# geonuklee/slam-toolkit

Measured on NVIDIA B200. Metric: orb_extract_match_stereo_frames_per_s, higher is better.
Workload: dtype u8

## Files before the change

slam-toolkit_b200/csrc/sfe_extract.cu:

```cuda
#include <cuda_fp16.h>

#include <algorithm>
#include <cmath>
#include <mutex>
#include <type_traits>

#include "sfe_extract.cuh"

namespace sfe {

__device__ __forceinline__ uint32_t ldg_word_at(const uint8_t *p) {
    const uintptr_t a = (uintptr_t)p;
    const uint32_t *w = (const uint32_t *)(a & ~(uintptr_t)3);
    return __funnelshift_r(__ldg(w), __ldg(w + 1), (uint32_t)(a & 3) * 8);
}

__device__ __forceinline__ uint32_t dp4a_u8u8(uint32_t a, uint32_t b, uint32_t c) {
    uint32_t d;
    asm("dp4a.u32.u32 %0, %1, %2, %3;" : "=r"(d) : "r"(a), "r"(b), "r"(c));
    return d;
}
__device__ __forceinline__ uint32_t dp2a_lo(uint32_t a, uint32_t b, uint32_t c) {
    uint32_t d;
    asm("dp2a.lo.u32.u32 %0, %1, %2, %3;" : "=r"(d) : "r"(a), "r"(b), "r"(c));
// ... 130 lines not shown
    uint32_t p[16], lo3[16], hi3[16];
#pragma unroll
    for (int k = 0; k < 16; k++) p[k] = __byte_perm(c0[off[k]], c1[off[k]], 0x5410);
#pragma unroll
    for (int s = 0; s < 16; s++) {
        lo3[s] = __vimin3_s16x2(p[s], p[(s + 1) & 15], p[(s + 2) & 15]);
        hi3[s] = __vimax3_s16x2(p[s], p[(s + 1) & 15], p[(s + 2) & 15]);
    }
    uint32_t max_of_min = 0u, min_of_max = 0x7fff7fffu;
#pragma unroll
    for (int s = 0; s < 16; s += 2) {
        const uint32_t l0 = __vimin3_s16x2(lo3[s], lo3[(s + 3) & 15], lo3[(s + 6) & 15]);
        const uint32_t l1 = __vimin3_s16x2(lo3[s + 1], lo3[(s + 4) & 15], lo3[(s + 7) & 15]);
        const uint32_t h0 = __vimax3_s16x2(hi3[s], hi3[(s + 3) & 15], hi3[(s + 6) & 15]);
        const uint32_t h1 = __vimax3_s16x2(hi3[s + 1], hi3[(s + 4) & 15], hi3[(s + 7) & 15]);
        max_of_min = __vimax3_s16x2(max_of_min, l0, l1);
        min_of_max = __vimin3_s16x2(min_of_max, h0, h1);
    }
    const int v0 = c0[0], v1 = c1[0];
    best0 = max(v0 - (int)(min_of_max & 0xFFFF), (int)(max_of_min & 0xFFFF) - v0);
    best1 = max(v1 - (int)(min_of_max >> 16), (int)(max_of_min >> 16) - v1);
}

template <bool kTma>
__global__ void __launch_bounds__(kFastThreads, kFastCtasPerSm) fast_segments_kernel(ImgSet S, FastPlan P, const SegRec *__restrict__ segs,
                                                                     const __grid_constant__ TmaMaps M) {
    constexpr int TP = kFastTilePitch, TW = TP / 4, SP = kFastScorePitch, T = kFastThreads;
    pdl_enter();
    extern __shared__ __align__(128) uint32_t fast_smem[];
    uint32_t *tile32 = fast_smem;
    uint8_t *score = (uint8_t *)(tile32 + P.tile_rows * TW);
    uint16_t *pre = (uint16_t *)(score + P.score_rows * SP);
    uint16_t *det = pre + P.list_cap;
    __shared__ int n_pre, n_det;
    __shared__ int cell_surv[kFastMaxCells];
    __shared__ uint64_t bar;
    const uint8_t *tile = (const uint8_t *)tile32;

    const uint4 rec = __ldg((const uint4 *)segs + blockIdx.x);
    const int ini_x = (short)(rec.x & 0xFFFF), ini_y = (short)(rec.x >> 16), tw = (short)(rec.y & 0xFFFF);
    const int sh = (rec.y >> 16) & 0xFF, level = rec.y >> 24, n_cells = rec.z & 0xFF, w_cell = (rec.z >> 8) & 0xFF;
    const int inv_w = rec.z >> 16, th = sh - 6;
    const FastLevel &F = P.lv[level];
    const int img = blockIdx.y, tid = threadIdx.x, lane = tid & 31, warp = tid >> 5;
    const int xa = (ini_x - 4) & ~15;
    const int cs = ini_x + 3 - xa;
    if (kTma) {
        if (tid == 0) {
            mbar_init(&bar, 1);
            mbar_expect_tx(&bar, (uint32_t)(P.tile_rows * TP));
            const bool set_a = img < S.split;
            const CUtensorMap *map = level == 0 ? (set_a ? &M.lv[0] : &M.l0b) : &M.lv[level];
            const int z = level == 0 ? S.in_z0 + (set_a ? img : img - S.split) : slot_of(S, img);
            tma_load_3d(tile32, map, &bar, xa, ini_y, z);
        }
    } else {
        const uint8_t *src;
        int pitch;
        if (level == 0) {
            pitch = S.in_pitch;
            src = img < S.split ? S.in_a + (size_t)img * S.in_stride : S.in_b + (size_t)(img - S.split) * S.in_stride;
        } else {
            pitch = F.pitch;
            src = S.pyr + (size_t)slot_of(S, img) * S.pyr_stride + F.plane_off;
        }
        src += (size_t)ini_y * pitch + xa;
        const int nw = min(((cs + tw - 1) >> 2) + 2, TW);
        for (int r = warp; r < sh; r += T / 32)
            for (int j = lane; j < nw; j += 32) tile32[r * TW + j] = ldg_word_at(src + (size_t)r * pitch + 4 * j);
    }
    const int jw = (cs >> 2) + lane, x0 = 4 * jw - cs;
    uint32_t vm = 0;
#pragma unroll
    for (int k = 0; k < 4; k++)
        if (x0 + k >= 0 && x0 + k < tw) vm |= 0x80u << (8 * k);
    uint32_t todo = (1u << n_cells) - 1;
    int t = P.ini_th;
    for (int i = tid; i < (th + 2) * (SP / 16); i += T) ((uint4 *)score)[i] = make_uint4(0, 0, 0, 0);
    for (int attempt = 0; attempt < 2; attempt++) {
        if (tid == 0) { n_pre = 0; n_det = 0; }
        if (tid < kFastMaxCells) cell_surv[tid] = 0;
        __syncthreads();
        if (kTma && attempt == 0) mbar_wait(&bar, 0);
        uint32_t vm_now = vm;
        if (attempt) {
#pragma unroll
            for (int k = 0; k < 4; k++)
                if (!((todo >> ((max(x0 + k, 0) * inv_w) >> 16)) & 1)) vm_now &= ~(0x80u << (8 * k));
        }
        const uint32_t kk = (uint32_t)(0x7F - min(t, 127)) * 0x01010101u;
        if (vm_now) {
            const uint32_t *row = tile32 + (warp + 3) * TW + jw;
            for (int y = warp; y < th; y += T / 32, row += (T / 32) * TW) {
                const uint32_t c = row[0];
                const uint32_t dv0 = __vabsdiffu4(row[-3 * TW], c), dv1 = __vabsdiffu4(row[3 * TW], c);
                const uint32_t dh0 = __vabsdiffu4(__byte_perm(row[-1], c, 0x4321), c);
                const uint32_t dh1 = __vabsdiffu4(__byte_perm(c, row[1], 0x6543), c);
                const uint32_t rv = (((dv0 | dv1) & 0x7F7F7F7Fu) + kk) | dv0 | dv1;
                const uint32_t rh = (((dh0 | dh1) & 0x7F7F7F7Fu) + kk) | dh0 | dh1;
                const uint32_t m = rv & rh & vm_now;
                if (m) {
                    int pos = atomicAdd(&n_pre, __popc(m));
                    const uint16_t item = (uint16_t)((y << 8) + x0);
                    if (m & 0x80u) pre[pos++] = item;
                    if (m & 0x8000u) pre[pos++] = item + 1;
                    if (m & 0x800000u) pre[pos++] = item + 2;
                    if (m & 0x80000000u) pre[pos] = item + 3;
                }
            }
        }
        __syncthreads();
        const int np = n_pre, npairs = (np + 1) >> 1;
        for (int e0 = 0; e0 < npairs; e0 += T) {
            bool corner0 = false, corner1 = false;
            uint16_t yx0 = 0, yx1 = 0;
            const int e = e0 + tid;
            if (e < npairs) {
                yx0 = pre[2 * e];
                yx1 = pre[min(2 * e + 1, np - 1)];
                int best0, best1;
                fast_best_x2<TP>(&tile[((yx0 >> 8) + 3) * TP + (yx0 & 255) + cs], &tile[((yx1 >> 8) + 3) * TP + (yx1 & 255) + cs],
                                 best0, best1);
                corner0 = best0 > t;
                corner1 = best1 > t && 2 * e + 1 < np;
                if (corner0) score[((yx0 >> 8) + 1) * SP + (yx0 & 255) + 1] = (uint8_t)best0;
                if (corner1) score[((yx1 >> 8) + 1) * SP + (yx1 & 255) + 1] = (uint8_t)best1;
            }
            const uint32_t c0 = __ballot_sync(0xffffffffu, corner0), c1 = __ballot_sync(0xffffffffu, corner1);
            if (c0 | c1) {
                int base = 0;
                if (lane == 0) base = atomicAdd(&n_det, __popc(c0) + __popc(c1));
                base = __shfl_sync(0xffffffffu, base, 0);
                const uint32_t lt = (1u << lane) - 1;
                if (corner0) det[base + __popc(c0 & lt)] = yx0;
                if (corner1) det[base + __popc(c0) + __popc(c1 & lt)] = yx1;
            }
        }
        __syncthreads();
        const int nd = n_det, slot = slot_of(S, img);
        uint32_t *out = S.cand + (size_t)slot * S.cand_stride + F.cand_off;
        for (int e0 = warp * 32; e0 < nd; e0 += T) {
            bool keep = false;
            uint32_t packed = 0;
            int cell = 0;
            if (e0 + lane < nd) {
                const uint16_t yx = det[e0 + lane];
                const int x = yx & 255, y = yx >> 8;
                cell = (x * inv_w) >> 16;
                const int cx0 = cell * w_cell, cx1 = min(cx0 + w_cell, tw);
                const uint8_t *sc = &score[(y + 1) * SP + x + 1];
                const int s = sc[0];
                const int lft = x > cx0 ? __vimax3_s32(sc[-1], sc[-SP - 1], sc[SP - 1]) : 0;
                const int rgt = x + 1 < cx1 ? __vimax3_s32(sc[1], sc[-SP + 1], sc[SP + 1]) : 0;
                keep = s > __vimax3_s32(max(sc[-SP], sc[SP]), lft, rgt);
                packed = (uint32_t)(s - 1) << 24 | (uint32_t)(ini_y - kBorder + y + 3) << 12 | (uint32_t)(ini_x - kBorder + x + 3);
            }
            const uint32_t kept = __ballot_sync(0xffffffffu, keep);
            if (kept) {
                int base = 0;
                if (lane == 0) base = atomicAdd(&S.cand_count[slot * S.nlevels + level], __popc(kept));
                base = __shfl_sync(0xffffffffu, base, 0);
                if (keep) {
                    const int o = base + __popc(kept & ((1u << lane) - 1));
                    if (o < F.cand_cap) out[o] = packed;
                    else atomicOr(&S.flags[slot], kFlagCandOverflow);
                    cell_surv[cell] = 1;
                }
            }
        }
        __syncthreads();
        const uint32_t retry = __ballot_sync(0xffffffffu, lane < n_cells && ((todo >> lane) & 1) && cell_surv[min(lane, kFastMaxCells - 1)] == 0);
        if (retry == 0 || P.min_th >= t) break;
        t = P.min_th;
        todo = retry;
        __syncthreads();
    }
}

template <bool kWide>
struct ONodeT {
    typedef typename std::conditional<kWide, uint32_t, unsigned short>::type pos_t;
    short x0, x1, y0, y1;
    pos_t start, cnt;
};

template <bool kWide>
struct OctSmemT {
    typedef ONodeT<kWide> ONode;
    typedef typename ONode::pos_t pos_t;
    uint32_t *pk[2];
    uint16_t *own[2];
    pos_t *qs;
    ONode *nd[2];
    uint16_t *eidx[2];
    uint32_t *child;
    uint16_t *childpos;
    int *tord;
    int *arr_a, *arr_b;
// ... 886 lines not shown
    }
}

}

using namespace sfe;

enum { kStagePyramid, kStageFast, kStageQuadtree, kStageBlur, kStageDescribe, kStageStereo, kStageTrack, kNumStages };
constexpr int kOctreeSmemCand = 3072;
constexpr int kComputeStreams = 4;
constexpr int kMaxChunks = 16;

struct sfe_extractor {
    int device = 0;
    cudaStream_t stream = nullptr;
    cudaStream_t s_h2d = nullptr, s_d2h = nullptr;
    cudaStream_t extra[kComputeStreams - 1] = {};
    int n_compute = 3;
    cudaStream_t aux[3] = {nullptr, nullptr, nullptr};
    cudaEvent_t ev_fork[3] = {}, ev_join[3] = {};
    int dev_split = 3;
    bool split_small = false;
    int octree_ctas = 0;
    int sm_count = 148;
    bool piped_now = false;
    bool orient_tma = true;
    bool overlap_tail = true;
    bool tail_pending = false;
    int overlap_blur = 2;
    cudaEvent_t ev_start = nullptr;
    bool async_dev = false;
    cudaEvent_t ev_in[kMaxChunks] = {}, ev_done[kMaxChunks] = {};
    int chunks_override = 0;
    bool trace = false;
    cudaEvent_t tr_ev[3 * kMaxChunks + 1] = {};
    sfe_extractor_params prm{};
    float scale[kMaxLevels], inv_scale[kMaxLevels], sigma2[kMaxLevels], inv_sigma2[kMaxLevels];
    int quota[kMaxLevels];
    int max_images = 0;
    int w = 0, h = 0;
    LevelPlan lv[kMaxLevels];
    FastPlan fast{};
    alignas(64) TmaMaps fast_maps{}, blur_maps{}, pyr_maps{};
    alignas(64) OrientMaps orient_maps{};
    int pyr_box_w = 0, pyr_box_h = 0;
    bool tma_plan_ok = false, tma_disabled = false, tma_now = false;
    const void *l0_key[2] = {nullptr, nullptr};
    size_t l0_geom[4] = {0, 0, 0, 0};
    int pitch0 = 0;
    std::vector<SegRec> segs;
    int seg_level_start[kMaxLevels + 1] = {};
    DevBuf<SegRec> d_segs;
    size_t fast_smem = 0, pyr_smem = 0;
    int pyr_wide_h[kMaxLevels] = {};
    std::vector<TilePlan> tiles;
    size_t pyr_stride = 0, blur_stride = 0;
    int cand_stride = 0, kpst_stride = 0, max_cand = 0, max_nodes = 0;
    size_t octree_smem = 0;
    int octree_smem_cand = 0, octree_slots = 0, octree_cand_override = 0;
    struct GraphEntry {
        uint64_t plan_gen = 0;
        int frames = 0, cap = 0, stereo = 0, seen = 0;
        double sp[3] = {0, 0, 0};
        const void *ptr[7] = {};
        cudaGraphExec_t exec = nullptr;
        int64_t launches = 0;
        uint64_t used = 0;
    };
    std::vector<GraphEntry> graphs;
    uint64_t plan_gen = 0, graph_clock = 0;
    bool use_graphs = true;
    bool use_pdl = true;
    bool octree_ff = true;
    bool pdl_now = false;
    bool octree_wide = false;
// ... 199 lines not shown
            for (int ty = 0; ty < L.h; ty += kPyrTileH) {
                const int last = std::min(ty + kPyrTileH, L.h) - 1;
                const int span = (int)(ytab[L.ytab_off + last].x >> 16) - (int)(ytab[L.ytab_off + ty].x & 0xFFFF) + 1;
                max_src_rows = std::max(max_src_rows, span);
            }
        }
    }
    ex->pyr_stride = std::max<size_t>(pyr_off, 128);
    ex->blur_stride = std::max<size_t>(blur_off, 128);
    ex->cand_stride = std::max(cand_off, 1);
    ex->kpst_stride = std::max(kp_off, 1);
    ex->max_cand = (std::max(max_cand, 1) + 7) & ~7;
    ex->max_nodes = max_nodes;
    ex->pyr_smem = (size_t)max_src_rows * kPyrTileW * sizeof(uint16_t);
    ex->pyr_box_w = (int)align_up((size_t)max_src_cols, 16);
    ex->pyr_box_h = max_src_rows;
    SFE_REQUIRE(ex->pyr_smem + (size_t)ex->pyr_box_w * ex->pyr_box_h <= 48 * 1024 && ex->pyr_box_w <= 256 && ex->pyr_box_h <= 256,
                SFE_ERR_UNSUPPORTED, "scale factor too large for the pyramid tile");
    ex->fast.nlevels = nl;
    ex->fast.ini_th = ex->prm.ini_th_fast;
    ex->fast.min_th = ex->prm.min_th_fast;
    ex->fast.n_segs = (int)ex->segs.size();
    ex->fast.tile_rows = (max_sh + 1) & ~1;
    ex->fast.score_rows = max_sh - 4;
    ex->fast.list_cap = (max_list + 7) & ~7;
    ex->fast_smem = (size_t)ex->fast.tile_rows * kFastTilePitch + (size_t)ex->fast.score_rows * kFastScorePitch + 2 * 2 * (size_t)ex->fast.list_cap;
    SFE_REQUIRE(ex->fast_smem <= 200 * 1024, SFE_ERR_UNSUPPORTED, "FAST segment working set exceeds shared memory");
    ex->octree_smem_cand = std::min(ex->max_cand, ex->octree_cand_override > 0 ? ex->octree_cand_override : kOctreeSmemCand) & ~7;
    if (ex->octree_smem_cand < 8) ex->octree_smem_cand = 8;
    ex->octree_wide = ex->max_cand > kNarrowCandCap;
    const size_t oct_cand_bytes = ex->octree_wide ? 16 : 14, oct_node_bytes = ex->octree_wide ? sizeof(ONodeT<true>) : sizeof(ONodeT<false>);
    ex->octree_smem = (size_t)ex->octree_smem_cand * oct_cand_bytes + (size_t)max_nodes * (16 + 3 * 4 + 2 * oct_node_bytes + 2 * 2 + 8) + 32 * 4 + 64;
    SFE_REQUIRE(ex->octree_smem <= 227 * 1024, SFE_ERR_UNSUPPORTED, "quadtree working set exceeds shared memory");
    {
        int big_levels = 0;
        for (int l = 0; l < nl; l++) big_levels += ex->lv[l].cand_cap > ex->octree_smem_cand;
        ex->octree_slots = big_levels * ex->max_images;
    }
    SFE_CUDA(ex->d_octree_scratch.ensure(std::max<size_t>((size_t)ex->octree_slots * ex->max_cand * oct_cand_bytes, 16)));
    const int n = ex->max_images;
    SFE_CUDA(ex->d_pyr.ensure(ex->pyr_stride * n));
    SFE_CUDA(ex->d_blur.ensure(ex->blur_stride * n));
    SFE_CUDA(ex->d_cand.ensure((size_t)ex->cand_stride * n));
    SFE_CUDA(ex->d_kpst.ensure((size_t)ex->kpst_stride * n));
    SFE_CUDA(ex->d_counts.ensure((size_t)n * (2 * nl + 1) + 1));
    SFE_CUDA(cudaMemsetAsync(ex->d_counts.p, 0, sizeof(int) * ex->d_counts.n, ex->stream));
    SFE_CUDA(ex->d_tiles.ensure(std::max<size_t>(ex->tiles.size(), 1)));
    SFE_CUDA(ex->d_segs.ensure(std::max<size_t>(ex->segs.size(), 1)));
    if (!ex->segs.empty())
        SFE_CUDA(cudaMemcpyAsync(ex->d_segs.p, ex->segs.data(), sizeof(SegRec) * ex->segs.size(), cudaMemcpyHostToDevice, ex->stream));
    SFE_CUDA(ex->d_xtab.ensure(std::max<size_t>(xtab.size(), 1)));
    SFE_CUDA(ex->d_ytab.ensure(std::max<size_t>(ytab.size(), 1)));
    if (!ex->tiles.empty())
        SFE_CUDA(cudaMemcpyAsync(ex->d_tiles.p, ex->tiles.data(), sizeof(TilePlan) * ex->tiles.size(), cudaMemcpyHostToDevice, ex->stream));
    if (!xtab.empty()) {
        SFE_CUDA(cudaMemcpyAsync(ex->d_xtab.p, xtab.data(), sizeof(uint2) * xtab.size(), cudaMemcpyHostToDevice, ex->stream));
        SFE_CUDA(cudaMemcpyAsync(ex->d_ytab.p, ytab.data(), sizeof(uint2) * ytab.size(), cudaMemcpyHostToDevice, ex->stream));
    }
    SFE_CUDA(cudaStreamSynchronize(ex->stream));
    ex->tma_plan_ok = !ex->tma_disabled;
    for (int l = 0; l < nl && ex->tma_plan_ok; l++) {
        const LevelPlan &L = ex->lv[l];
        if (L.w < 8 || L.h < 8) ex->tma_plan_ok = false;
        if (l == 0 || !ex->tma_plan_ok) continue;
        ex->tma_plan_ok = tma_encode_u8_3d(&ex->fast_maps.lv[l], ex->d_pyr.p + L.plane_off, L.w, L.h, n, L.pitch, ex->pyr_stride,
                                           kFastTilePitch, ex->fast.tile_rows) &&
                          tma_encode_u8_3d(&ex->blur_maps.lv[l], ex->d_pyr.p + L.plane_off, L.w, L.h, n, L.pitch, ex->pyr_stride,
                                           kBlurInWords * 4, kBlurTileH + 6) &&
                          (nl < 2 || tma_encode_u8_3d(&ex->pyr_maps.lv[l], ex->d_pyr.p + L.plane_off, L.w, L.h, n, L.pitch, ex->pyr_stride,
                                                      ex->pyr_box_w, ex->pyr_box_h)) &&
                          tma_encode_u8_3d(&ex->orient_maps.ic[l], ex->d_pyr.p + L.plane_off, L.w, L.h, n, L.pitch, ex->pyr_stride,
// ... 97 lines not shown
        const bool ok = tma_encode_u8_3d(&ex->fast_maps.lv[0], a, L.w, L.h, n_a, pitch, stride, kFastTilePitch, ex->fast.tile_rows) &&
                        tma_encode_u8_3d(&ex->fast_maps.l0b, b, L.w, L.h, n_b, pitch, stride, kFastTilePitch, ex->fast.tile_rows) &&
                        tma_encode_u8_3d(&ex->blur_maps.lv[0], a, L.w, L.h, n_a, pitch, stride, kBlurInWords * 4, kBlurTileH + 6) &&
                        tma_encode_u8_3d(&ex->blur_maps.l0b, b, L.w, L.h, n_b, pitch, stride, kBlurInWords * 4, kBlurTileH + 6) &&
                        (ex->prm.nlevels < 2 ||
                         (tma_encode_u8_3d(&ex->pyr_maps.lv[0], a, L.w, L.h, n_a, pitch, stride, ex->pyr_box_w, ex->pyr_box_h) &&
                          tma_encode_u8_3d(&ex->pyr_maps.l0b, b, L.w, L.h, n_b, pitch, stride, ex->pyr_box_w, ex->pyr_box_h))) &&
                        tma_encode_u8_3d(&ex->orient_maps.ic[0], a, L.w, L.h, n_a, pitch, stride, kIcBoxW, kIcBoxH) &&
                        tma_encode_u8_3d(&ex->orient_maps.ic_l0b, b, L.w, L.h, n_b, pitch, stride, kIcBoxW, kIcBoxH);
        ex->l0_key[0] = ok ? a : nullptr;
        ex->l0_key[1] = ok ? b : nullptr;
        memcpy(ex->l0_geom, geom, sizeof(geom));
        if (!ok) return;
    }
    ex->tma_now = true;
}

constexpr bool kFastTma = true;

static int launch_fast(sfe_extractor *ex, cudaStream_t st, const ImgSet &S, int count, int level0 = 0, int level1 = kMaxLevels) {
    level1 = std::min(level1, ex->prm.nlevels);
    const int seg0 = ex->seg_level_start[level0], nseg = ex->seg_level_start[level1] - seg0;
    if (nseg <= 0) return SFE_OK;
    const dim3 grid((unsigned)nseg, count);
    if (ex->fast_smem > 48 * 1024) {
        static std::mutex mu;
        static size_t granted[64] = {};
        std::lock_guard<std::mutex> lock(mu);
        if (ex->fast_smem > granted[ex->device & 63]) {
            SFE_CUDA(cudaFuncSetAttribute(fast_segments_kernel<true>, cudaFuncAttributeMaxDynamicSharedMemorySize, (int)ex->fast_smem));
            SFE_CUDA(cudaFuncSetAttribute(fast_segments_kernel<false>, cudaFuncAttributeMaxDynamicSharedMemorySize, (int)ex->fast_smem));
            granted[ex->device & 63] = ex->fast_smem;
        }
    }
    {
        static std::once_flag once[64];
        std::call_once(once[ex->device & 63], [] {
            cudaFuncSetAttribute(fast_segments_kernel<true>, cudaFuncAttributePreferredSharedMemoryCarveout, cudaSharedmemCarveoutMaxShared);
            cudaFuncSetAttribute(fast_segments_kernel<false>, cudaFuncAttributePreferredSharedMemoryCarveout, cudaSharedmemCarveoutMaxShared);
        });
    }
    if (ex->tma_now && kFastTma)
        launch_k(fast_segments_kernel<true>, grid, kFastThreads, ex->fast_smem, st, ex->pdl_now, S, ex->fast, ex->d_segs.p + seg0, ex->fast_maps);
    else
        launch_k(fast_segments_kernel<false>, grid, kFastThreads, ex->fast_smem, st, ex->pdl_now, S, ex->fast, ex->d_segs.p + seg0, ex->fast_maps);
    return SFE_OK;
}

constexpr int kSplitMaxImages = 4;

static int join_tail(sfe_extractor *ex) {
    if (ex->tail_pending) {
        SFE_CUDA(cudaStreamWaitEvent(ex->stream, ex->ev_join[1], 0));
        ex->tail_pending = false;
    }
    return SFE_OK;
}

static int enqueue_extract(sfe_extractor *ex, cudaStream_t st, const ImgSet &S, int count, const OutSet &O) {
    const int nl = ex->prm.nlevels;
    prof_mark(ex, 0);
    auto launch_pyr = [&](int l) {
        const LevelPlan &D = ex->lv[l], &Q = ex->lv[l - 1];
        const PyrStep P{D.w, D.h, D.pitch, D.plane_off, Q.w, l == 1 ? S.in_pitch : Q.pitch, Q.plane_off, l == 1, D.xtab_off, D.ytab_off,
                        l - 1, ex->pyr_box_w, ex->pyr_box_h, ex->pyr_wide_h[l]};
        dim3 grid(div_up(D.w, kPyrTileW), div_up(D.h, kPyrTileH), count);
        if (ex->tma_now)
            launch_k(pyr_resize_kernel<true>, grid, 256, ex->pyr_smem + (size_t)ex->pyr_box_w * ex->pyr_box_h, st, ex->pdl_now, S, P, ex->d_xtab.p,
// ... 536 lines not shown
        set_error("stream/event creation: %s", cudaGetErrorString(cudaGetLastError()));
        sfe_extractor_destroy(ex);
        return SFE_ERR_CUDA;
    }
    if (const char *env = getenv("SFE_PIPELINE_CHUNKS")) ex->chunks_override = atoi(env);
    if (const char *env = getenv("SFE_NO_TMA")) ex->tma_disabled = atoi(env) != 0;
    if (const char *env = getenv("SFE_OVERLAP_BLUR")) ex->overlap_blur = atoi(env);
    cudaDeviceGetAttribute(&ex->sm_count, cudaDevAttrMultiProcessorCount, device);
    if (const char *env = getenv("SFE_OCTREE_CTAS")) ex->octree_ctas = atoi(env);
    if (const char *env = getenv("SFE_ORIENT_TMA")) ex->orient_tma = atoi(env) != 0;
    if (const char *env = getenv("SFE_OVERLAP_TAIL")) ex->overlap_tail = atoi(env) != 0;
    if (const char *env = getenv("SFE_TRACE")) ex->trace = atoi(env) != 0;
    if (const char *env = getenv("SFE_COMPUTE_STREAMS")) ex->n_compute = std::max(1, std::min(atoi(env), kComputeStreams));
    if (ex->trace)
        for (auto &e : ex->tr_ev) cudaEventCreate(&e);
    if (const char *env = getenv("SFE_OCTREE_SMEM_CAND")) ex->octree_cand_override = atoi(env);
    if (const char *env = getenv("SFE_CAND_CAP")) ex->cand_cap_override = std::max(8, atoi(env));
    if (const char *env = getenv("SFE_GRAPHS")) ex->use_graphs = atoi(env) != 0;
    if (const char *env = getenv("SFE_PDL")) ex->use_pdl = atoi(env) != 0;
    if (const char *env = getenv("SFE_OCTREE_FF")) ex->octree_ff = atoi(env) != 0;
    if (const char *env = getenv("SFE_COPY_KERNEL")) ex->use_copy_kernel = atoi(env) != 0;
    if (const char *env = getenv("SFE_SPLIT_SMALL")) ex->split_small = atoi(env) != 0;
    if (const char *env = getenv("SFE_DEV_SPLIT")) ex->dev_split = std::max(1, std::min(atoi(env), kComputeStreams));
    build_tables(ex);
    *out = ex;
    return SFE_OK;
}

int sfe_extractor_destroy(sfe_extractor *ex) {
    if (!ex) return SFE_OK;
    drop_graphs(ex);
    if (ex->h_flags_pinned) cudaFreeHost(ex->h_flags_pinned);
    if (ex->h_stage) cudaFreeHost(ex->h_stage);
    DeviceGuard g(ex->device);
    SFE_REQUIRE(g.ok, SFE_ERR_NO_DEVICE, "cannot select the handle's device");
    cudaStreamSynchronize(ex->stream);
    ex->d_pyr.release(); ex->d_blur.release(); ex->d_in.release(); ex->d_l0.release(); ex->d_octree_scratch.release(); ex->d_desc.release();
    ex->d_cand.release(); ex->d_kpst.release(); ex->d_counts.release();
    ex->d_tiles.release(); ex->d_segs.release(); ex->d_xtab.release(); ex->d_ytab.release();
    ex->d_kps.release(); ex->d_nout.release(); ex->d_sidx.release(); ex->d_sdist.release(); ex->d_tidx.release(); ex->d_tdist.release();
    ex->track.cell_start.release(); ex->track.order.release(); ex->track.valid.release(); ex->track.sxy.release(); ex->track.sdesc.release(); ex->track.best.release();
    for (int i = 0; i <= kNumStages; i++)
        if (ex->prof_ev[i]) cudaEventDestroy(ex->prof_ev[i]);
    for (int i = 0; i < kMaxChunks; i++) {
        if (ex->ev_in[i]) cudaEventDestroy(ex->ev_in[i]);
        if (ex->ev_done[i]) cudaEventDestroy(ex->ev_done[i]);
    }
    for (auto &e : ex->tr_ev)
        if (e) cudaEventDestroy(e);
    for (int i = 0; i < 3; i++) {
        if (ex->ev_fork[i]) cudaEventDestroy(ex->ev_fork[i]);
        if (ex->ev_join[i]) cudaEventDestroy(ex->ev_join[i]);
        if (ex->aux[i]) cudaStreamDestroy(ex->aux[i]);
    }
    if (ex->ev_start) cudaEventDestroy(ex->ev_start);
    for (auto &e : ex->extra)
        if (e) cudaStreamDestroy(e);
    if (ex->s_h2d) cudaStreamDestroy(ex->s_h2d);
    if (ex->s_d2h) cudaStreamDestroy(ex->s_d2h);
    cudaStreamDestroy(ex->stream);
    delete ex;
    return SFE_OK;
// ... 105 lines not shown
    int rc = sfe_extract_batch(ex, image, (size_t)stride * (h > 0 ? h : 0), 1, w, h, stride, kps, desc, cap, &n);
    *n_out = n;
    return rc;
}

static int stereo_frames_dev_once(sfe_extractor *ex, const uint8_t *left_dev, const uint8_t *right_dev, size_t image_stride,
                                  int frames, int w, int h, int stride, const sfe_stereo_params *sp, const sfe_track_params *tp,
                                  sfe_keypoint *kps_l_dev, uint8_t *desc_l_dev, int32_t *n_l_dev, sfe_keypoint *kps_r_dev,
                                  uint8_t *desc_r_dev, int32_t *n_r_dev, int32_t *stereo_idx_dev, int32_t *stereo_dist_dev,
                                  int32_t *track_idx_dev, int32_t *track_dist_dev, int cap) {
    int rc = prepare(ex, 2 * frames, w, h, stride, cap);
    if (rc != SFE_OK) return rc;
    if (!sp) sp = &k_default_stereo;
    const OutSet O{kps_l_dev, kps_r_dev, desc_l_dev, desc_r_dev, n_l_dev, n_r_dev, cap};
    const ImgSet S = make_imgset(ex, left_dev, right_dev, frames, image_stride, stride);
    prepare_l0_maps(ex, left_dev, right_dev, frames, frames, image_stride, stride);
    if ((rc = reset_counters(ex)) != SFE_OK) return rc;
    const int nsplit = !ex->profiling && frames >= 16 * ex->dev_split ? std::min(ex->dev_split, ex->n_compute) : 1;
    if (nsplit <= 1) {
        if ((rc = enqueue_extract(ex, ex->stream, S, 2 * frames, O)) != SFE_OK) return rc;
    } else {
        SFE_CUDA(cudaEventRecord(ex->ev_start, ex->stream));
        for (int c = 1; c < nsplit; c++) SFE_CUDA(cudaStreamWaitEvent(ex->extra[c - 1], ex->ev_start, 0));
        for (int c = nsplit - 1; c >= 0; c--) {
            const int f0 = (int)((long long)frames * c / nsplit), f1 = (int)((long long)frames * (c + 1) / nsplit);
            cudaStream_t sc = c == 0 ? ex->stream : ex->extra[c - 1];
            if ((rc = enqueue_extract(ex, sc, chunk_of(S, f0, f1, true), 2 * (f1 - f0), chunk_of(O, f0))) != SFE_OK) return rc;
            if (c > 0) SFE_CUDA(cudaEventRecord(ex->ev_done[c], sc));
        }
        for (int c = 1; c < nsplit; c++) SFE_CUDA(cudaStreamWaitEvent(ex->stream, ex->ev_done[c], 0));
    }
    const bool tail = ex->async_dev && ex->overlap_tail && !ex->profiling;
    cudaStream_t sm = tail ? ex->aux[1] : ex->stream;
    if (!tail) {
        if ((rc = join_tail(ex)) != SFE_OK) return rc;
    } else if (tp && ex->tail_pending && (size_t)frames * cap > ex->track.best.n) {
        SFE_CUDA(cudaStreamSynchronize(ex->aux[1]));
    }
    if (tail) {
        SFE_CUDA(cudaEventRecord(ex->ev_fork[1], ex->stream));
        SFE_CUDA(cudaStreamWaitEvent(sm, ex->ev_fork[1], 0));
    }
    launch_stereo_match(sm, frames, cap, kps_l_dev, desc_l_dev, n_l_dev, kps_r_dev, desc_r_dev, n_r_dev, sp->y_threshold,
                        sp->max_dx, sp->best12_threshold, stereo_idx_dev, stereo_dist_dev);
    prof_mark(ex, 6);
    ex->prof_has_stereo = true;
    ex->launches++;
    SFE_CUDA(cudaGetLastError());
    if (tp) {
        if ((rc = launch_track_frames(sm, ex->device, ex->track, frames, cap, kps_l_dev, desc_l_dev, n_l_dev, kps_r_dev,
                                      stereo_idx_dev, *tp, track_idx_dev, track_dist_dev)) != SFE_OK)
            return rc;
// ... 229 lines not shown
```

slam-toolkit_b200/csrc/sfe_extract.cuh:

```cuda
#pragma once
#include "sfe_common.cuh"
#include "sfe_tma.cuh"

namespace sfe {

constexpr int kMaxLevels = 16;
constexpr int kEdge = 19;
constexpr int kBorder = kEdge - 3;
constexpr int kHalfPatch = 15;
constexpr int kMaxSub = 66;
constexpr int kNarrowCandCap = 60000;
constexpr int kMaxCandCap = 1 << 22;
constexpr int kBlurTileW = 128, kBlurTileH = 32;
constexpr int kBlurInWords = 40;
constexpr int kBlurLead = 16;

struct LevelPlan {
    int w, h, pitch;
    int plane_off;
    int blur_pitch, blur_off;
    int win_w, win_h;
    int n_cols, n_rows, w_cell, h_cell;
    int quota;
    int n_ini;
// ... 4 lines not shown
    int xtab_off, ytab_off;
    float scale;
    float size;
};

struct SegRec {
    short ini_x, ini_y;
    short tw;
    unsigned char sh, level;
    unsigned char n_cells, w_cell;
    unsigned short inv_w;
    unsigned int pad;
};
static_assert(sizeof(SegRec) == 16, "SegRec is loaded as one uint4");
struct FastLevel {
    int pitch, plane_off;
    int cand_off, cand_cap;
};
struct FastPlan {
    FastLevel lv[kMaxLevels];
    int nlevels, n_cells, n_segs;
    int ini_th, min_th;
    int tile_rows, score_rows, list_cap;
};
constexpr int kFastThreads = 256;
constexpr int kFastCtasPerSm = 5;
#ifndef SFE_FAST_TILE_PITCH
#define SFE_FAST_TILE_PITCH 176
#endif
constexpr int kFastTilePitch = SFE_FAST_TILE_PITCH;
constexpr int kFastScorePitch = 144;
constexpr int kFastSegPx = 128;
constexpr int kFastMaxCells = 8;

struct TilePlan {
    short level, x0, y0, pad;
};

struct ImgSet {
    const uint8_t *in_a, *in_b;
    size_t in_stride;
    int in_pitch;
    int split;
    int in_z0;
    int slot_a, slot_b;
    uint8_t *pyr;
// ... 59 lines not shown
```

Baseline: 68210.

## Make FAST segment kernel persistent with double-buffered TMA prefetch and sparse score clearing

```diff
diff --git a/slam-toolkit_b200/csrc/sfe_extract.cu b/slam-toolkit_b200/csrc/sfe_extract.cu
--- a/slam-toolkit_b200/csrc/sfe_extract.cu
+++ b/slam-toolkit_b200/csrc/sfe_extract.cu
@@ -176,158 +176,196 @@
     best1 = max(v1 - (int)(min_of_max >> 16), (int)(max_of_min >> 16) - v1);
 }
 
+__device__ __forceinline__ void fast_issue_box(const ImgSet &S, const FastPlan &P, const SegRec *__restrict__ segs, int seg, int img,
+                                               const TmaMaps &M, uint32_t *dst, uint64_t *bar) {
+    const uint32_t x = __ldg((const uint32_t *)(segs + seg)), y = __ldg((const uint32_t *)(segs + seg) + 1);
+    const int ini_x = (short)(x & 0xFFFF), ini_y = (short)(x >> 16), level = y >> 24;
+    const bool set_a = img < S.split;
+    const CUtensorMap *map = level == 0 ? (set_a ? &M.lv[0] : &M.l0b) : &M.lv[level];
+    const int z = level == 0 ? S.in_z0 + (set_a ? img : img - S.split) : slot_of(S, img);
+    mbar_expect_tx(bar, (uint32_t)(P.tile_rows * kFastTilePitch));
+    tma_load_3d(dst, map, bar, (ini_x - 4) & ~15, ini_y, z);
+}
+
 template <bool kTma>
 __global__ void __launch_bounds__(kFastThreads, kFastCtasPerSm) fast_segments_kernel(ImgSet S, FastPlan P, const SegRec *__restrict__ segs,
+                                                                     int nseg, int count, int *__restrict__ work,
                                                                      const __grid_constant__ TmaMaps M) {
     constexpr int TP = kFastTilePitch, TW = TP / 4, SP = kFastScorePitch, T = kFastThreads;
     pdl_enter();
     extern __shared__ __align__(128) uint32_t fast_smem[];
-    uint32_t *tile32 = fast_smem;
-    uint8_t *score = (uint8_t *)(tile32 + P.tile_rows * TW);
+    uint8_t *score = (uint8_t *)fast_smem + 2 * P.tile_buf;
     uint16_t *pre = (uint16_t *)(score + P.score_rows * SP);
     uint16_t *det = pre + P.list_cap;
     __shared__ int n_pre, n_det;
     __shared__ int cell_surv[kFastMaxCells];
-    __shared__ uint64_t bar;
-    const uint8_t *tile = (const uint8_t *)tile32;
-
-    const uint4 rec = __ldg((const uint4 *)segs + blockIdx.x);
-    const int ini_x = (short)(rec.x & 0xFFFF), ini_y = (short)(rec.x >> 16), tw = (short)(rec.y & 0xFFFF);
-    const int sh = (rec.y >> 16) & 0xFF, level = rec.y >> 24, n_cells = rec.z & 0xFF, w_cell = (rec.z >> 8) & 0xFF;
-    const int inv_w = rec.z >> 16, th = sh - 6;
-    const FastLevel &F = P.lv[level];
-    const int img = blockIdx.y, tid = threadIdx.x, lane = tid & 31, warp = tid >> 5;
-    const int xa = (ini_x - 4) & ~15;
-    const int cs = ini_x + 3 - xa;
-    if (kTma) {
+    __shared__ uint64_t bar[2];
+    __shared__ int2 next_item[2];
+    const int tid = threadIdx.x, lane = tid & 31, warp = tid >> 5, items = nseg * count;
+    const bool more = (int)gridDim.x < items;
+    const int2 first = make_int2(blockIdx.x % nseg, blockIdx.x / nseg);
+    int drawn = items;
+    if (tid == 0) {
+        if (kTma) {
+            mbar_init(&bar[0], 1);
+            if (more) mbar_init(&bar[1], 1);
+            if (first.y < count) fast_issue_box(S, P, segs, first.x, first.y, M, fast_smem, &bar[0]);
+        }
+        if (more) drawn = (int)gridDim.x + atomicAdd(work, 1);
+    }
+    for (int i = tid; i < P.score_rows * (SP / 16); i += T) ((uint4 *)score)[i] = make_uint4(0, 0, 0, 0);
+    int n_run = 0;
+    for (int2 item = first; item.y < count; item = next_item[n_run & 1], n_run++) {
+        const int buf = kTma ? n_run & 1 : 0;
+        uint32_t *tile32 = (uint32_t *)((uint8_t *)fast_smem + buf * P.tile_buf);
+        const uint8_t *tile = (const uint8_t *)tile32;
+        const int seg = item.x, img = item.y;
+        const uint4 rec = __ldg((const uint4 *)segs + seg);
+        const int ini_x = (short)(rec.x & 0xFFFF), ini_y = (short)(rec.x >> 16), tw = (short)(rec.y & 0xFFFF);
+        const int sh = (rec.y >> 16) & 0xFF, level = rec.y >> 24, n_cells = rec.z & 0xFF, w_cell = (rec.z >> 8) & 0xFF;
+        const int inv_w = rec.z >> 16, th = sh - 6;
+        const FastLevel &F = P.lv[level];
+        const int xa = (ini_x - 4) & ~15;
+        const int cs = ini_x + 3 - xa;
         if (tid == 0) {
-            mbar_init(&bar, 1);
-            mbar_expect_tx(&bar, (uint32_t)(P.tile_rows * TP));
-            const bool set_a = img < S.split;
-            const CUtensorMap *map = level == 0 ? (set_a ? &M.lv[0] : &M.l0b) : &M.lv[level];
-            const int z = level == 0 ? S.in_z0 + (set_a ? img : img - S.split) : slot_of(S, img);
-            tma_load_3d(tile32, map, &bar, xa, ini_y, z);
-        }
-    } else {
-        const uint8_t *src;
-        int pitch;
-        if (level == 0) {
-            pitch = S.in_pitch;
-            src = img < S.split ? S.in_a + (size_t)img * S.in_stride : S.in_b + (size_t)(img - S.split) * S.in_stride;
-        } else {
-            pitch = F.pitch;
-            src = S.pyr + (size_t)slot_of(S, img) * S.pyr_stride + F.plane_off;
-        }
-        src += (size_t)ini_y * pitch + xa;
-        const int nw = min(((cs + tw - 1) >> 2) + 2, TW);
-        for (int r = warp; r < sh; r += T / 32)
-            for (int j = lane; j < nw; j += 32) tile32[r * TW + j] = ldg_word_at(src + (size_t)r * pitch + 4 * j);
-    }
-    const int jw = (cs >> 2) + lane, x0 = 4 * jw - cs;
-    uint32_t vm = 0;
+            const int2 next = drawn < items ? make_int2(drawn % nseg, drawn / nseg) : make_int2(0, count);
+            next_item[n_run & 1] = next;
+            if (next.y < count) {
+                if (kTma) {
+                    asm volatile("fence.proxy.async.shared::cta;" ::: "memory");
+                    fast_issue_box(S, P, segs, next.x, next.y, M, (uint32_t *)((uint8_t *)fast_smem + (buf ^ 1) * P.tile_buf), &bar[buf ^ 1]);
+                }
+                drawn = (int)gridDim.x + atomicAdd(work, 1);
+            }
+        }
+        if (!kTma) {
+            const uint8_t *src;
+            int pitch;
+            if (level == 0) {
+                pitch = S.in_pitch;
+                src = img < S.split ? S.in_a + (size_t)img * S.in_stride : S.in_b + (size_t)(img - S.split) * S.in_stride;
+            } else {
+                pitch = F.pitch;
+                src = S.pyr + (size_t)slot_of(S, img) * S.pyr_stride + F.plane_off;
+            }
+            src += (size_t)ini_y * pitch + xa;
+            const int nw = min(((cs + tw - 1) >> 2) + 2, TW);
+            for (int r = warp; r < sh; r += T / 32)
+                for (int j = lane; j < nw; j += 32) tile32[r * TW + j] = ldg_word_at(src + (size_t)r * pitch + 4 * j);
+        }
+        const int jw = (cs >> 2) + lane, x0 = 4 * jw - cs;
+        uint32_t vm = 0;
 #pragma unroll
-    for (int k = 0; k < 4; k++)
-        if (x0 + k >= 0 && x0 + k < tw) vm |= 0x80u << (8 * k);
-    uint32_t todo = (1u << n_cells) - 1;
-    int t = P.ini_th;
-    for (int i = tid; i < (th + 2) * (SP / 16); i += T) ((uint4 *)score)[i] = make_uint4(0, 0, 0, 0);
-    for (int attempt = 0; attempt < 2; attempt++) {
-        if (tid == 0) { n_pre = 0; n_det = 0; }
-        if (tid < kFastMaxCells) cell_surv[tid] = 0;
-        __syncthreads();
-        if (kTma && attempt == 0) mbar_wait(&bar, 0);
-        uint32_t vm_now = vm;
-        if (attempt) {
+        for (int k = 0; k < 4; k++)
+            if (x0 + k >= 0 && x0 + k < tw) vm |= 0x80u << (8 * k);
+        uint32_t todo = (1u << n_cells) - 1;
+        int t = P.ini_th;
+#ifdef SFE_FAST_EAGER_CLEAR
+        if (n_run) for (int i = tid; i < (th + 2) * (SP / 16); i += T) ((uint4 *)score)[i] = make_uint4(0, 0, 0, 0);
+#endif
+        for (int attempt = 0; attempt < 2; attempt++) {
+            if (tid == 0) { n_pre = 0; n_det = 0; }
+            __syncthreads();
+            if (tid < kFastMaxCells) cell_surv[tid] = 0;
+            if (kTma && attempt == 0) mbar_wait(&bar[buf], (n_run >> 1) & 1);
+            uint32_t vm_now = vm;
+            if (attempt) {
 #pragma unroll
-            for (int k = 0; k < 4; k++)
-                if (!((todo >> ((max(x0 + k, 0) * inv_w) >> 16)) & 1)) vm_now &= ~(0x80u << (8 * k));
-        }
-        const uint32_t kk = (uint32_t)(0x7F - min(t, 127)) * 0x01010101u;
-        if (vm_now) {
-            const uint32_t *row = tile32 + (warp + 3) * TW + jw;
-            for (int y = warp; y < th; y += T / 32, row += (T / 32) * TW) {
-                const uint32_t c = row[0];
-                const uint32_t dv0 = __vabsdiffu4(row[-3 * TW], c), dv1 = __vabsdiffu4(row[3 * TW], c);
-                const uint32_t dh0 = __vabsdiffu4(__byte_perm(row[-1], c, 0x4321), c);
-                const uint32_t dh1 = __vabsdiffu4(__byte_perm(c, row[1], 0x6543), c);
-                const uint32_t rv = (((dv0 | dv1) & 0x7F7F7F7Fu) + kk) | dv0 | dv1;
-                const uint32_t rh = (((dh0 | dh1) & 0x7F7F7F7Fu) + kk) | dh0 | dh1;
-                const uint32_t m = rv & rh & vm_now;
-                if (m) {
-                    int pos = atomicAdd(&n_pre, __popc(m));
-                    const uint16_t item = (uint16_t)((y << 8) + x0);
-                    if (m & 0x80u) pre[pos++] = item;
-                    if (m & 0x8000u) pre[pos++] = item + 1;
-                    if (m & 0x800000u) pre[pos++] = item + 2;
-                    if (m & 0x80000000u) pre[pos] = item + 3;
+                for (int k = 0; k < 4; k++)
+                    if (!((todo >> ((max(x0 + k, 0) * inv_w) >> 16)) & 1)) vm_now &= ~(0x80u << (8 * k));
+            }
+            const uint32_t kk = (uint32_t)(0x7F - min(t, 127)) * 0x01010101u;
+            if (vm_now) {
+                const uint32_t *row = tile32 + (warp + 3) * TW + jw;
+                for (int y = warp; y < th; y += T / 32, row += (T / 32) * TW) {
+                    const uint32_t c = row[0];
+                    const uint32_t dv0 = __vabsdiffu4(row[-3 * TW], c), dv1 = __vabsdiffu4(row[3 * TW], c);
+                    const uint32_t dh0 = __vabsdiffu4(__byte_perm(row[-1], c, 0x4321), c);
+                    const uint32_t dh1 = __vabsdiffu4(__byte_perm(c, row[1], 0x6543), c);
+                    const uint32_t rv = (((dv0 | dv1) & 0x7F7F7F7Fu) + kk) | dv0 | dv1;
+                    const uint32_t rh = (((dh0 | dh1) & 0x7F7F7F7Fu) + kk) | dh0 | dh1;
+                    const uint32_t m = rv & rh & vm_now;
+                    if (m) {
+                        int pos = atomicAdd(&n_pre, __popc(m));
+                        const uint16_t yx = (uint16_t)((y << 8) + x0);
+                        if (m & 0x80u) pre[pos++] = yx;
+                        if (m & 0x8000u) pre[pos++] = yx + 1;
+                        if (m & 0x800000u) pre[pos++] = yx + 2;
+                        if (m & 0x80000000u) pre[pos] = yx + 3;
+                    }
                 }
             }
-        }
-        __syncthreads();
-        const int np = n_pre, npairs = (np + 1) >> 1;
-        for (int e0 = 0; e0 < npairs; e0 += T) {
-            bool corner0 = false, corner1 = false;
-            uint16_t yx0 = 0, yx1 = 0;
-            const int e = e0 + tid;
-            if (e < npairs) {
-                yx0 = pre[2 * e];
-                yx1 = pre[min(2 * e + 1, np - 1)];
-                int best0, best1;
-                fast_best_x2<TP>(&tile[((yx0 >> 8) + 3) * TP + (yx0 & 255) + cs], &tile[((yx1 >> 8) + 3) * TP + (yx1 & 255) + cs],
-                                 best0, best1);
-                corner0 = best0 > t;
-                corner1 = best1 > t && 2 * e + 1 < np;
-                if (corner0) score[((yx0 >> 8) + 1) * SP + (yx0 & 255) + 1] = (uint8_t)best0;
-                if (corner1) score[((yx1 >> 8) + 1) * SP + (yx1 & 255) + 1] = (uint8_t)best1;
-            }
-            const uint32_t c0 = __ballot_sync(0xffffffffu, corner0), c1 = __ballot_sync(0xffffffffu, corner1);
-            if (c0 | c1) {
-                int base = 0;
-                if (lane == 0) base = atomicAdd(&n_det, __popc(c0) + __popc(c1));
-                base = __shfl_sync(0xffffffffu, base, 0);
-                const uint32_t lt = (1u << lane) - 1;
-                if (corner0) det[base + __popc(c0 & lt)] = yx0;
-                if (corner1) det[base + __popc(c0) + __popc(c1 & lt)] = yx1;
-            }
-        }
-        __syncthreads();
-        const int nd = n_det, slot = slot_of(S, img);
-        uint32_t *out = S.cand + (size_t)slot * S.cand_stride + F.cand_off;
-        for (int e0 = warp * 32; e0 < nd; e0 += T) {
-            bool keep = false;
-            uint32_t packed = 0;
-            int cell = 0;
-            if (e0 + lane < nd) {
-                const uint16_t yx = det[e0 + lane];
-                const int x = yx & 255, y = yx >> 8;
-                cell = (x * inv_w) >> 16;
-                const int cx0 = cell * w_cell, cx1 = min(cx0 + w_cell, tw);
-                const uint8_t *sc = &score[(y + 1) * SP + x + 1];
-                const int s = sc[0];
-                const int lft = x > cx0 ? __vimax3_s32(sc[-1], sc[-SP - 1], sc[SP - 1]) : 0;
-                const int rgt = x + 1 < cx1 ? __vimax3_s32(sc[1], sc[-SP + 1], sc[SP + 1]) : 0;
-                keep = s > __vimax3_s32(max(sc[-SP], sc[SP]), lft, rgt);
-                packed = (uint32_t)(s - 1) << 24 | (uint32_t)(ini_y - kBorder + y + 3) << 12 | (uint32_t)(ini_x - kBorder + x + 3);
-            }
-            const uint32_t kept = __ballot_sync(0xffffffffu, keep);
-            if (kept) {
-                int base = 0;
-                if (lane == 0) base = atomicAdd(&S.cand_count[slot * S.nlevels + level], __popc(kept));
-                base = __shfl_sync(0xffffffffu, base, 0);
-                if (keep) {
-                    const int o = base + __popc(kept & ((1u << lane) - 1));
-                    if (o < F.cand_cap) out[o] = packed;
-                    else atomicOr(&S.flags[slot], kFlagCandOverflow);
-                    cell_surv[cell] = 1;
+            __syncthreads();
+            const int np = n_pre, npairs = (np + 1) >> 1;
+            for (int e0 = 0; e0 < npairs; e0 += T) {
+                bool corner0 = false, corner1 = false;
+                uint16_t yx0 = 0, yx1 = 0;
+                const int e = e0 + tid;
+                if (e < npairs) {
+                    yx0 = pre[2 * e];
+                    yx1 = pre[min(2 * e + 1, np - 1)];
+                    int best0, best1;
+                    fast_best_x2<TP>(&tile[((yx0 >> 8) + 3) * TP + (yx0 & 255) + cs], &tile[((yx1 >> 8) + 3) * TP + (yx1 & 255) + cs],
+                                     best0, best1);
+                    corner0 = best0 > t;
+                    corner1 = best1 > t && 2 * e + 1 < np;
+                    if (corner0) score[((yx0 >> 8) + 1) * SP + (yx0 & 255) + 1] = (uint8_t)best0;
+                    if (corner1) score[((yx1 >> 8) + 1) * SP + (yx1 & 255) + 1] = (uint8_t)best1;
                 }
-            }
-        }
-        __syncthreads();
-        const uint32_t retry = __ballot_sync(0xffffffffu, lane < n_cells && ((todo >> lane) & 1) && cell_surv[min(lane, kFastMaxCells - 1)] == 0);
-        if (retry == 0 || P.min_th >= t) break;
-        t = P.min_th;
-        todo = retry;
-        __syncthreads();
+                const uint32_t c0 = __ballot_sync(0xffffffffu, corner0), c1 = __ballot_sync(0xffffffffu, corner1);
+                if (c0 | c1) {
+                    int base = 0;
+                    if (lane == 0) base = atomicAdd(&n_det, __popc(c0) + __popc(c1));
+                    base = __shfl_sync(0xffffffffu, base, 0);
+                    const uint32_t lt = (1u << lane) - 1;
+                    if (corner0) det[base + __popc(c0 & lt)] = yx0;
+                    if (corner1) det[base + __popc(c0) + __popc(c1 & lt)] = yx1;
+                }
+            }
+            __syncthreads();
+            const int nd = n_det, slot = slot_of(S, img);
+            uint32_t *out = S.cand + (size_t)slot * S.cand_stride + F.cand_off;
+            for (int e0 = warp * 32; e0 < nd; e0 += T) {
+                bool keep = false;
+                uint32_t packed = 0;
+                int cell = 0;
+                if (e0 + lane < nd) {
+                    const uint16_t yx = det[e0 + lane];
+                    const int x = yx & 255, y = yx >> 8;
+                    cell = (x * inv_w) >> 16;
+                    const int cx0 = cell * w_cell, cx1 = min(cx0 + w_cell, tw);
+                    const uint8_t *sc = &score[(y + 1) * SP + x + 1];
+                    const int s = sc[0];
+                    const int lft = x > cx0 ? __vimax3_s32(sc[-1], sc[-SP - 1], sc[SP - 1]) : 0;
+                    const int rgt = x + 1 < cx1 ? __vimax3_s32(sc[1], sc[-SP + 1], sc[SP + 1]) : 0;
+                    keep = s > __vimax3_s32(max(sc[-SP], sc[SP]), lft, rgt);
+                    packed = (uint32_t)(s - 1) << 24 | (uint32_t)(ini_y - kBorder + y + 3) << 12 | (uint32_t)(ini_x - kBorder + x + 3);
+                }
+                const uint32_t kept = __ballot_sync(0xffffffffu, keep);
+                if (kept) {
+                    int base = 0;
+                    if (lane == 0) base = atomicAdd(&S.cand_count[slot * S.nlevels + level], __popc(kept));
+                    base = __shfl_sync(0xffffffffu, base, 0);
+                    if (keep) {
+                        const int o = base + __popc(kept & ((1u << lane) - 1));
+                        if (o < F.cand_cap) out[o] = packed;
+                        else atomicOr(&S.flags[slot], kFlagCandOverflow);
+                        cell_surv[cell] = 1;
+                    }
+                }
+            }
+            __syncthreads();
+            const uint32_t retry = __ballot_sync(0xffffffffu, lane < n_cells && ((todo >> lane) & 1) && cell_surv[min(lane, kFastMaxCells - 1)] == 0);
+#ifndef SFE_FAST_EAGER_CLEAR
+            for (int e = tid; e < nd; e += T) {
+                const uint16_t yx = det[e];
+                score[((yx >> 8) + 1) * SP + (yx & 255) + 1] = 0;
+            }
+#endif
+            if (retry == 0 || P.min_th >= t) break;
+            t = P.min_th;
+            todo = retry;
+        }
     }
 }
 
@@ -1260,6 +1298,12 @@
     int dev_split = 3;
     bool split_small = false;
     int octree_ctas = 0;
+    bool fast_persistent = true;
+    int fast_ctas = 0;
+    int fast_share = 1;
+    int fast_slots[2] = {};
+    size_t fast_slots_smem = 0;
+    int fast_share_exp = 0;
     int sm_count = 148;
     bool piped_now = false;
     bool orient_tma = true;
@@ -1289,6 +1333,7 @@
     std::vector<SegRec> segs;
     int seg_level_start[kMaxLevels + 1] = {};
     DevBuf<SegRec> d_segs;
+    DevBuf<int> d_fast_work;
     size_t fast_smem = 0, pyr_smem = 0;
     int pyr_wide_h[kMaxLevels] = {};
     std::vector<TilePlan> tiles;
@@ -1534,9 +1579,10 @@
     ex->fast.min_th = ex->prm.min_th_fast;
     ex->fast.n_segs = (int)ex->segs.size();
     ex->fast.tile_rows = (max_sh + 1) & ~1;
+    ex->fast.tile_buf = (int)align_up((size_t)ex->fast.tile_rows * kFastTilePitch, 128);
     ex->fast.score_rows = max_sh - 4;
     ex->fast.list_cap = (max_list + 7) & ~7;
-    ex->fast_smem = (size_t)ex->fast.tile_rows * kFastTilePitch + (size_t)ex->fast.score_rows * kFastScorePitch + 2 * 2 * (size_t)ex->fast.list_cap;
+    ex->fast_smem = 2 * (size_t)ex->fast.tile_buf + (size_t)ex->fast.score_rows * kFastScorePitch + 2 * 2 * (size_t)ex->fast.list_cap;
     SFE_REQUIRE(ex->fast_smem <= 200 * 1024, SFE_ERR_UNSUPPORTED, "FAST segment working set exceeds shared memory");
     ex->octree_smem_cand = std::min(ex->max_cand, ex->octree_cand_override > 0 ? ex->octree_cand_override : kOctreeSmemCand) & ~7;
     if (ex->octree_smem_cand < 8) ex->octree_smem_cand = 8;
@@ -1559,6 +1605,7 @@
     SFE_CUDA(cudaMemsetAsync(ex->d_counts.p, 0, sizeof(int) * ex->d_counts.n, ex->stream));
     SFE_CUDA(ex->d_tiles.ensure(std::max<size_t>(ex->tiles.size(), 1)));
     SFE_CUDA(ex->d_segs.ensure(std::max<size_t>(ex->segs.size(), 1)));
+    SFE_CUDA(ex->d_fast_work.ensure(kComputeStreams + 1));
     if (!ex->segs.empty())
         SFE_CUDA(cudaMemcpyAsync(ex->d_segs.p, ex->segs.data(), sizeof(SegRec) * ex->segs.size(), cudaMemcpyHostToDevice, ex->stream));
     SFE_CUDA(ex->d_xtab.ensure(std::max<size_t>(xtab.size(), 1)));
@@ -1702,7 +1749,6 @@
     level1 = std::min(level1, ex->prm.nlevels);
     const int seg0 = ex->seg_level_start[level0], nseg = ex->seg_level_start[level1] - seg0;
     if (nseg <= 0) return SFE_OK;
-    const dim3 grid((unsigned)nseg, count);
     if (ex->fast_smem > 48 * 1024) {
         static std::mutex mu;
         static size_t granted[64] = {};
@@ -1720,10 +1766,35 @@
             cudaFuncSetAttribute(fast_segments_kernel<false>, cudaFuncAttributePreferredSharedMemoryCarveout, cudaSharedmemCarveoutMaxShared);
         });
     }
-    if (ex->tma_now && kFastTma)
-        launch_k(fast_segments_kernel<true>, grid, kFastThreads, ex->fast_smem, st, ex->pdl_now, S, ex->fast, ex->d_segs.p + seg0, ex->fast_maps);
+    const bool tma = ex->tma_now && kFastTma;
+    if (ex->fast_slots_smem != ex->fast_smem) {
+        for (int i = 0; i < 2; i++) {
+            int per_sm = 0;
+            SFE_CUDA(cudaOccupancyMaxActiveBlocksPerMultiprocessor(&per_sm, i ? fast_segments_kernel<true> : fast_segments_kernel<false>,
+                                                                   kFastThreads, ex->fast_smem));
+            ex->fast_slots[i] = std::max(per_sm, 1) * ex->sm_count;
+        }
+        ex->fast_slots_smem = ex->fast_smem;
+    }
+    const int items = nseg * count;
+    if (getenv("SFE_FAST_DEBUG")) fprintf(stderr, "fast: items %d slots %d/%d share %d smem %zu\n", nseg * count, ex->fast_slots[0], ex->fast_slots[1], ex->fast_share, ex->fast_smem);
+    const int slots = ex->fast_ctas > 0 ? ex->fast_ctas : std::max(ex->fast_slots[tma] / ex->fast_share, 1);
+    const int grid = ex->fast_persistent ? std::min(items, slots) : items;
+    int *work = nullptr;
+    if (grid < items) {
+        int wi = 0;
+        for (int i = 0; i < kComputeStreams - 1; i++)
+            if (st == ex->extra[i]) wi = 1 + i;
+        if (st == ex->aux[2]) wi = kComputeStreams;
+        work = ex->d_fast_work.p + wi;
+        SFE_CUDA(cudaMemsetAsync(work, 0, sizeof(int), st));
+    }
+    if (tma)
+        launch_k(fast_segments_kernel<true>, grid, kFastThreads, ex->fast_smem, st, ex->pdl_now, S, ex->fast, ex->d_segs.p + seg0, nseg, count, work,
+                 ex->fast_maps);
     else
-        launch_k(fast_segments_kernel<false>, grid, kFastThreads, ex->fast_smem, st, ex->pdl_now, S, ex->fast, ex->d_segs.p + seg0, ex->fast_maps);
+        launch_k(fast_segments_kernel<false>, grid, kFastThreads, ex->fast_smem, st, ex->pdl_now, S, ex->fast, ex->d_segs.p + seg0, nseg, count, work,
+                 ex->fast_maps);
     return SFE_OK;
 }
 
@@ -2306,6 +2377,9 @@
     if (const char *env = getenv("SFE_COPY_KERNEL")) ex->use_copy_kernel = atoi(env) != 0;
     if (const char *env = getenv("SFE_SPLIT_SMALL")) ex->split_small = atoi(env) != 0;
     if (const char *env = getenv("SFE_DEV_SPLIT")) ex->dev_split = std::max(1, std::min(atoi(env), kComputeStreams));
+    if (const char *env = getenv("SFE_FAST_PERSISTENT")) ex->fast_persistent = atoi(env) != 0;
+    if (const char *env = getenv("SFE_FAST_CTAS")) ex->fast_ctas = atoi(env);
+    if (const char *env = getenv("SFE_FAST_SHARE_EXP")) ex->fast_share_exp = atoi(env);
     build_tables(ex);
     *out = ex;
     return SFE_OK;
@@ -2321,7 +2395,7 @@
     cudaStreamSynchronize(ex->stream);
     ex->d_pyr.release(); ex->d_blur.release(); ex->d_in.release(); ex->d_l0.release(); ex->d_octree_scratch.release(); ex->d_desc.release();
     ex->d_cand.release(); ex->d_kpst.release(); ex->d_counts.release();
-    ex->d_tiles.release(); ex->d_segs.release(); ex->d_xtab.release(); ex->d_ytab.release();
+    ex->d_tiles.release(); ex->d_segs.release(); ex->d_fast_work.release(); ex->d_xtab.release(); ex->d_ytab.release();
     ex->d_kps.release(); ex->d_nout.release(); ex->d_sidx.release(); ex->d_sdist.release(); ex->d_tidx.release(); ex->d_tdist.release();
     ex->track.cell_start.release(); ex->track.order.release(); ex->track.valid.release(); ex->track.sxy.release(); ex->track.sdesc.release(); ex->track.best.release();
     for (int i = 0; i <= kNumStages; i++)
@@ -2473,12 +2547,15 @@
     } else {
         SFE_CUDA(cudaEventRecord(ex->ev_start, ex->stream));
         for (int c = 1; c < nsplit; c++) SFE_CUDA(cudaStreamWaitEvent(ex->extra[c - 1], ex->ev_start, 0));
+        ex->fast_share = ex->fast_share_exp ? nsplit : 1;
         for (int c = nsplit - 1; c >= 0; c--) {
             const int f0 = (int)((long long)frames * c / nsplit), f1 = (int)((long long)frames * (c + 1) / nsplit);
             cudaStream_t sc = c == 0 ? ex->stream : ex->extra[c - 1];
-            if ((rc = enqueue_extract(ex, sc, chunk_of(S, f0, f1, true), 2 * (f1 - f0), chunk_of(O, f0))) != SFE_OK) return rc;
+            rc = enqueue_extract(ex, sc, chunk_of(S, f0, f1, true), 2 * (f1 - f0), chunk_of(O, f0));
+            if (rc != SFE_OK) { ex->fast_share = 1; return rc; }
             if (c > 0) SFE_CUDA(cudaEventRecord(ex->ev_done[c], sc));
         }
+        ex->fast_share = 1;
         for (int c = 1; c < nsplit; c++) SFE_CUDA(cudaStreamWaitEvent(ex->stream, ex->ev_done[c], 0));
     }
     const bool tail = ex->async_dev && ex->overlap_tail && !ex->profiling;
diff --git a/slam-toolkit_b200/csrc/sfe_extract.cuh b/slam-toolkit_b200/csrc/sfe_extract.cuh
--- a/slam-toolkit_b200/csrc/sfe_extract.cuh
+++ b/slam-toolkit_b200/csrc/sfe_extract.cuh
@@ -50,6 +50,7 @@
     int nlevels, n_cells, n_segs;
     int ini_th, min_th;
     int tile_rows, score_rows, list_cap;
+    int tile_buf;
 };
 constexpr int kFastThreads = 256;
 constexpr int kFastCtasPerSm = 5;
```

Result: slower. 67130, median of 6 (-1.6%).
